# dernasherbrezon/sdr-server

Measured on AMD Instinct MI355X. Metric: input IQ Msamples/s processed (all clients), 2.016 Msps->48 kHz xlating FIR, higher is better.
Workload: dtype f32; 1 GPU; 1024 clients x 48 kHz off one 2.016 Msps cu8 stream, D=42, 505 taps, 262144-byte blocks (BASELINE configs[3]; N=1: the >=1000-client single-GPU target); clients_total=1024, clients_per_gpu=1024, blocks_per_call=8, mode=optimized, parallelism=single GPU, rccl_ranks=1, feed=xlating_multi (C host)

## Files before the change

### sdr-server_amd/csrc/xl_kernels.hip

```cpp
#include "xl_dev_inline.h"
#include "xl_chain_plan.h"

#include <hip/hip_ext.h>

#include <stdlib.h>

__global__ __launch_bounds__(64) void xl_nco_table_kernel(const XlNcoClient *__restrict__ cl, uint32_t n,
                                                          const float2 *state_in, float2 *state_out,
                                                          float2 *__restrict__ tab, const XlPos pos,
                                                          const uint32_t explicit_K, const uint32_t prio,
                                                          const uint32_t lanes) {
  if (prio == 3) __builtin_amdgcn_s_setprio(3);
  else if (prio == 2) __builtin_amdgcn_s_setprio(2);
  else if (prio == 1) __builtin_amdgcn_s_setprio(1);
  if (threadIdx.x >= lanes) return;
  const uint32_t c = blockIdx.x * lanes + threadIdx.x;
  if (c >= n) return;
  const XlNcoClient k = cl[c];
  const XlBnd bnd = xl_nco_bnd(k, pos, explicit_K);
  asm volatile("" ::: "v255", "a255");
  xl_nco_client_chain<true>(k, bnd, 0u, bnd.K, state_in, state_out, tab);
}

#define XLC_RING 64u
XL_DEV uint32_t xl_lds_off(const void *p) { return (uint32_t)(uintptr_t)(__attribute__((address_space(3))) const char *)p; }
XL_DEV void xl_lds_post(const uint32_t addr, const uint32_t v) { asm volatile("ds_write_b32 %0, %1" ::"v"(addr), "v"(v) : "memory"); }
XL_DEV void xl_lds_post64(const uint32_t addr, const v2f v) { asm volatile("ds_write_b64 %0, %1" ::"v"(addr), "v"(v) : "memory"); }
XL_DEV uint32_t xl_lds_poll(const uint32_t addr) {
  uint32_t v;
  asm volatile("ds_read_b32 %0, %1\n\ts_waitcnt lgkmcnt(0)" : "=v"(v) : "v"(addr) : "memory");
  return v;
}

XL_DEV uint32_t xl_lds_poll3_min(const uint32_t a0, const uint32_t a1, const uint32_t a2) {
  uint32_t v0, v1, v2;
  asm volatile("ds_read_b32 %0, %3\n\tds_read_b32 %1, %4\n\tds_read_b32 %2, %5\n\ts_waitcnt lgkmcnt(0)"
               : "=&v"(v0), "=&v"(v1), "=&v"(v2)
               : "v"(a0), "v"(a1), "v"(a2)
               : "memory");
  v0 = v0 < v1 ? v0 : v1;
  return v0 < v2 ? v0 : v2;
}
XL_DEV uint32_t xl_chain_lim(const uint32_t mn) { return mn >= 0x7FFFFFE0u ? 0xFFFFFFFFu : 2u * mn + XLC_RING; }
XL_DEV uint32_t xl_chain_wait_drained(const uint32_t upto, const uint32_t a0, const uint32_t a1, const uint32_t a2) {
  uint32_t lim = 0u;
  for (uint32_t spin = 0; spin < (1u << 22); ++spin) {
    lim = xl_chain_lim((uint32_t)__builtin_amdgcn_readfirstlane((int)xl_lds_poll3_min(a0, a1, a2)));
    if (upto <= lim) break;
    __builtin_amdgcn_s_sleep(1);
  }
  return lim;
}
XL_DEV uint32_t xl_chain_event(uint32_t ev) {
  const unsigned long long act = __ballot(ev != 0xFFFFFFFFu);
  if (act == 0ull) return 0xFFFFFFFFu;
  const uint32_t first = (uint32_t)__builtin_amdgcn_readlane((int)ev, (int)__ffsll((long long)act) - 1);
  if (__ballot(ev != 0xFFFFFFFFu && ev != first) == 0ull) return first;
#pragma unroll
  for (int sh = 1; sh < 64; sh <<= 1) {
    const uint32_t other = (uint32_t)__shfl_xor((int)ev, sh);
    ev = other < ev ? other : ev;
  }
  return (uint32_t)__builtin_amdgcn_readfirstlane((int)ev);
}

#define XLC_ALIGN ".p2align 6\n\t"
#define XLC_MUL "v_pk_mul_f32 %[t1], %[p], %[inc] op_sel_hi:[1,0]\n\tv_pk_mul_f32 %[t2], %[p], %[inc] op_sel:[0,1] op_sel_hi:[1,1]\n\t"
#define XLC_ADD "v_pk_add_f32 %[p], %[t1], %[t2] op_sel:[0,1] op_sel_hi:[1,0] neg_lo:[0,1]\n\t"
#define XLC_STEP XLC_MUL XLC_ADD
#define XLC_STEP2(I1, I2) XLC_MUL I1 "\n\t" XLC_ADD I2 "\n\t"
#define XLC_STEPS10 XLC_STEP XLC_STEP XLC_STEP XLC_STEP XLC_STEP XLC_STEP XLC_STEP XLC_STEP XLC_STEP XLC_STEP
#define XLC_ANY_LOOP                                                                       \
  "1:\n\t" XLC_MUL "ds_write_b64 %[addr], %[p]\n\t" XLC_ADD                               \
  XLC_STEP2("v_add_u32 %[cnt], 1, %[cnt]", "s_sub_u32 %[todo], %[todo], 1")               \
  XLC_MUL "ds_write_b32 %[paddr], %[cnt]\n\t" XLC_ADD                                     \
  XLC_MUL "v_add_u32 %[off], 0x200, %[off]\n\t" XLC_ADD                                   \
  XLC_MUL "v_and_b32 %[off], 0x7fff, %[off]\n\t" XLC_ADD                                  \
  XLC_STEP2("v_add_u32 %[addr], %[off], %[base]", "s_cmp_lg_u32 %[todo], 0")              \
  XLC_STEPS10 "s_cbranch_scc1 1b\n\t"
#define XLC_B8_LOOP                                                                        \
  "2:\n\t" XLC_E7("0", "512", "1024", "1536", "2048", "2560", "3072")                    \
  XLC_MUL "ds_write_b64 %[addr], %[p] offset:3584\n\t" XLC_ADD                           \
  XLC_STEP2("v_add_u32 %[cnt], 8, %[cnt]", "s_sub_u32 %[todo8], %[todo8], 1")            \
  XLC_MUL "ds_write_b32 %[paddr], %[cnt]\n\t" XLC_ADD                                    \
  XLC_MUL "v_add_u32 %[off], 0x1000, %[off]\n\t" XLC_ADD                                 \
  XLC_MUL "v_and_b32 %[off], 0x7fff, %[off]\n\t" XLC_ADD                                 \
  XLC_STEP2("v_add_u32 %[addr], %[off], %[base]", "s_cmp_lg_u32 %[todo8], 0")            \
  XLC_STEPS10 "s_cbranch_scc1 2b\n\t"
#define XLC_ANY_PART "s_cmp_eq_u32 %[todo], 0\n\ts_cbranch_scc1 3f\n\t" XLC_ANY_LOOP "3:\n\ts_nop 0\n\t"
#define XLC_B8_PART "s_cmp_eq_u32 %[todo8], 0\n\ts_cbranch_scc1 4f\n\t" XLC_B8_LOOP "4:\n\ts_nop 0\n\t"
#define XLC_STEP_LOOP "1:\n\t" XLC_STEP2("s_sub_u32 %[todo], %[todo], 1", "s_cmp_lg_u32 %[todo], 0") "s_cbranch_scc1 1b\n\t"
#define XLC_QENTRY(OFFS) XLC_MUL "ds_write_b64 %[addr], %[p] offset:" OFFS "\n\t" XLC_ADD XLC_STEP XLC_STEP
#define XLC_E(OFFS) XLC_QENTRY(OFFS) XLC_STEP XLC_STEP XLC_STEP XLC_STEPS10
#define XLC_E7(B0, B1, B2, B3, B4, B5, B6) XLC_E(B0) XLC_E(B1) XLC_E(B2) XLC_E(B3) XLC_E(B4) XLC_E(B5) XLC_E(B6)
#define XLC_E8(B0, B1, B2, B3, B4, B5, B6, B7) XLC_E7(B0, B1, B2, B3, B4, B5, B6) XLC_E(B7)
#define XLC_B32_LOOP                                                                                         \
  XLC_E8("0", "512", "1024", "1536", "2048", "2560", "3072", "3584")                                       \
  XLC_E8("4096", "4608", "5120", "5632", "6144", "6656", "7168", "7680")                                   \
  XLC_E8("8192", "8704", "9216", "9728", "10240", "10752", "11264", "11776")                               \
  XLC_E("12288") XLC_E("12800") XLC_E("13312") XLC_E("13824") XLC_E("14336") XLC_E("14848")               \
  XLC_QENTRY("15360")                                                                                      \
  XLC_MUL "ds_read_b32 %[mn], %[an0]\n\t" XLC_ADD                                                           \
  XLC_MUL "ds_read_b32 %[n1], %[an1]\n\t" XLC_ADD                                                           \
  XLC_MUL "ds_read_b32 %[n2], %[an2]\n\t" XLC_ADD XLC_STEPS10                                               \
  XLC_MUL "ds_write_b64 %[addr], %[p] offset:15872\n\t" XLC_ADD                                             \
  XLC_MUL "v_add_u32 %[cnt], 32, %[cnt]\n\t" XLC_ADD "s_sub_u32 %[todo], %[todo], 1\n\t"                    \
  XLC_MUL "ds_write_b32 %[paddr], %[cnt]\n\t" XLC_ADD                                                       \
  XLC_MUL "v_add_u32 %[off], 0x4000, %[off]\n\t" XLC_ADD                                                    \
  XLC_MUL "v_and_b32 %[off], 0x7fff, %[off]\n\t" XLC_ADD                                                    \
  XLC_STEP2("v_add_u32 %[addr], %[off], %[base]", "s_add_u32 %[need], %[need], 16")                         \
  XLC_STEP2("s_waitcnt lgkmcnt(0)", "v_min_u32 %[mn], %[mn], %[n1]")                                        \
  XLC_STEP2("v_min_u32 %[mn], %[mn], %[n2]", "s_nop 0")                                                     \
  XLC_STEP2("v_readfirstlane_b32 %[sm], %[mn]", "s_nop 0")                                                  \
  XLC_STEP2("s_cmp_ge_u32 %[sm], %[need]", "s_cselect_b32 %[st], %[todo], 0")                               \
  XLC_STEP XLC_STEP XLC_STEP XLC_STEP XLC_STEP XLC_STEP
static_assert(XL_PH_STRIDE == 16u && XLC_RING * 64u * 8u == 0x8000u, "the chain wave's asm blocks are written for 16 steps per entry and a 32 KB ring");

__global__ __launch_bounds__(256) void xl_nco_chain_kernel(const XlNcoClient *__restrict__ cl, uint32_t n,
                                                           const float2 *state_in, const XlChainCalls calls,
                                                           XlPos pos, unsigned long long *stats) {
  asm volatile("" ::: "v255", "a255");
  const unsigned long long t_entry = stats ? wall_clock64() : 0ull;
  __shared__ v2f ring[XLC_RING][64];
  __shared__ uint32_t s_emax;
  __shared__ uint32_t s_prod;
  __shared__ uint32_t s_next[3];
  const uint32_t w = __builtin_amdgcn_readfirstlane(threadIdx.x >> 6), lane = threadIdx.x & 63u;
  const uint32_t c = blockIdx.x * 64u + lane;
  const bool have = c < n;
  XlNcoClient k;
  k.incr = make_float2(1.0f, 0.0f);
  k.out_off = 0u, k.slot = 0u, k.D = 1u, k.rem0 = 0u;
  if (have) k = cl[c];
  v2f p = {1.0f, 0.0f};
  if (w == 0 && have) p = (v2f){state_in[k.slot].x, state_in[k.slot].y};
  unsigned long long cyc = 0ull, ticks = 0ull, wfirst = 0ull;
  uint32_t entries = 0u;
  for (uint32_t call = 0; call < calls.n; ++call, pos = xl_grid_next(pos)) {
    float2 *const tab = calls.tab[call];
    float2 *const state_out = calls.state_out[call];
    if (call) __syncthreads();
    XlBnd bnd = xl_nco_bnd(k, pos, 0xFFFFFFFFu);
    if (!have) bnd.K = 0u;
    const uint32_t K = bnd.K, E = (K + XL_PH_STRIDE - 1u) >> XL_PH_SHIFT;
    if (threadIdx.x == 0) {
      s_emax = 0u;
      s_prod = 0u;
      s_next[0] = 0u, s_next[1] = 1u, s_next[2] = 2u;
    }
    __syncthreads();
    if (w == 0 && E > 0u) atomicMax(&s_emax, E);
    __syncthreads();
    const uint32_t Emax = (uint32_t)__builtin_amdgcn_readfirstlane((int)s_emax);
    const uint32_t a_prod = xl_lds_off(&s_prod), a_ring0 = xl_lds_off(&ring[0][0]), a_ring = xl_lds_off(&ring[0][lane]);
    v2f *__restrict__ o = reinterpret_cast<v2f *>(tab) + (k.out_off >> XL_PH_SHIFT);
    if (w == 0) {
      __builtin_amdgcn_s_setprio(3);
      const v2f inc = {k.incr.x, k.incr.y};
      uint32_t nb = xl_bnd_next(bnd, 0u);
      const uint32_t a_n0 = xl_lds_off(&s_next[0]), a_n1 = xl_lds_off(&s_next[1]), a_n2 = xl_lds_off(&s_next[2]);
      const unsigned long long c0 = stats ? clock64() : 0ull, w0 = stats ? wall_clock64() : 0ull;
      unsigned long long t_region = 0ull, t_drain = 0ull, t_b32 = 0ull;
      uint32_t n_drain = 0u, n_b32 = 0u, n_event = 0u, n_runs = 0u;
      uint32_t e = 0;
      uint32_t lim = XLC_RING;
      uint32_t evs = xl_chain_event(0u < K ? (nb < K ? nb : K) : 0xFFFFFFFFu);
      while (e < Emax) {
        uint32_t e_stop = evs == 0u ? 0u : (evs - 1u) >> XL_PH_SHIFT;
        e_stop = e_stop < Emax ? e_stop : Emax;
        if (pos.pad & XL_POS_FMA_STEP) e_stop = e;
        const unsigned long long r0 = stats ? clock64() : 0ull;
        if ((e << XL_PH_SHIFT) < K) {
          const XlChainPlan8 pl = xl_chain_plan8(e, e_stop, XLC_RING, 32u, 8u);
          uint32_t ee = e;
          v2f t1, t2;
#define XLC_COVER_RUN(N1, N8, PARTS)                                                                                         \
  if ((N1) + (N8) != 0u) {                                                                                                   \
    uint32_t todo = (N1), todo8 = (N8);                                                                                      \
    const uint32_t total = todo + 8u * todo8;                                                                                \
    if (ee + total > lim) {                                                                                                  \
      const unsigned long long d0 = stats ? clock64() : 0ull;                                                                \
      lim = xl_chain_wait_drained(ee + total, a_n0, a_n1, a_n2);                                                             \
      if (stats) t_drain += clock64() - d0, ++n_drain;                                                                       \
    }                                                                                                                        \
    uint32_t off = ((ee & (XLC_RING - 1u)) << 9) + lane * (uint32_t)sizeof(v2f);     \
    uint32_t addr = a_ring0 + off, cnt = ee;                                                                                 \
    ee += total;                                                                                                             \
    asm volatile(XLC_ALIGN PARTS                                                                                             \
                 : [p] "+v"(p), [off] "+v"(off), [addr] "+v"(addr), [cnt] "+v"(cnt), [t1] "=&v"(t1), [t2] "=&v"(t2),         \
                   [todo] "+s"(todo), [todo8] "+s"(todo8)                                                                    \
                 : [inc] "v"(inc), [base] "v"(a_ring0), [paddr] "v"(a_prod)                                                  \
                 : "memory", "scc");                                                                                         \
  }
          XLC_COVER_RUN(pl.head1, pl.head8, XLC_ANY_PART XLC_B8_PART);
          for (uint32_t want = pl.blocks; want != 0u;) {
            if (ee + 32u > lim) {
              const unsigned long long d0 = stats ? clock64() : 0ull;
              lim = xl_chain_wait_drained(ee + 32u, a_n0, a_n1, a_n2);
              if (stats) t_drain += clock64() - d0, ++n_drain;
            }
            uint32_t off = ((ee & (XLC_RING - 1u)) << 9) + lane * (uint32_t)sizeof(v2f);
            uint32_t addr = a_ring0 + off, cnt = ee;
            uint32_t left = want, need = (ee >> 1) - 16u, mn, n1, n2, sm, st;
            const unsigned long long b0 = stats ? clock64() : 0ull;
            asm volatile(XLC_ALIGN "1:\n\t" XLC_B32_LOOP "s_cmp_lg_u32 %[st], 0\n\ts_cbranch_scc1 1b\n\t"
                         : [p] "+v"(p), [off] "+v"(off), [addr] "+v"(addr), [cnt] "+v"(cnt), [t1] "=&v"(t1), [t2] "=&v"(t2),
                           [mn] "=&v"(mn), [n1] "=&v"(n1), [n2] "=&v"(n2), [todo] "+s"(left), [need] "+s"(need), [sm] "=&s"(sm),
                           [st] "=&s"(st)
                         : [inc] "v"(inc), [base] "v"(a_ring0), [paddr] "v"(a_prod), [an0] "v"(a_n0), [an1] "v"(a_n1), [an2] "v"(a_n2)
                         : "memory", "scc");
            const uint32_t ran = (want - left) << 5;
            if (stats) t_b32 += clock64() - b0, n_b32 += ran, ++n_runs;
            lim = xl_chain_lim(sm);
            ee += ran;
            want = left;
          }
          XLC_COVER_RUN(pl.tail1, pl.tail8, XLC_B8_PART XLC_ANY_PART);
#undef XLC_COVER_RUN
        }
        if (e_stop > e) e = e_stop;
        if (stats) t_region += clock64() - r0, ++n_event;
        if (e < Emax) {
          if (e + 1u > lim) lim = xl_chain_wait_drained(e + 1u, a_n0, a_n1, a_n2);
          const uint32_t m0 = e << XL_PH_SHIFT;
          if (m0 < K) xl_lds_post64(a_ring + (e & (XLC_RING - 1u)) * 64u * (uint32_t)sizeof(v2f), p);
          xl_lds_post(a_prod, e + 1u);
          uint32_t m = m0;
          if (!(pos.pad & XL_POS_FMA_STEP) && evs - m0 - 1u < XL_PH_STRIDE &&
              __ballot(m0 < K && (nb != evs || m0 + XL_PH_STRIDE > K)) == 0ull && m0 < K) {
            v2f t1, t2;
            uint32_t todo = evs - m0;
            asm volatile(XLC_ALIGN XLC_STEP_LOOP
                         : [p] "+v"(p), [t1] "=&v"(t1), [t2] "=&v"(t2), [todo] "+s"(todo)
                         : [inc] "v"(inc)
                         : "scc");
            p = xl_nco_renorm(p);
            nb = xl_bnd_next(bnd, evs);
            m = evs;
            todo = m0 + XL_PH_STRIDE - evs;
            if (todo != 0u && __ballot(nb <= m0 + XL_PH_STRIDE) == 0ull) {
              asm volatile(XLC_ALIGN XLC_STEP_LOOP
                           : [p] "+v"(p), [t1] "=&v"(t1), [t2] "=&v"(t2), [todo] "+s"(todo)
                           : [inc] "v"(inc)
                           : "scc");
              m = m0 + XL_PH_STRIDE;
            }
          }
          for (; m < m0 + XL_PH_STRIDE && m < K; ++m) {
            p = xl_nco_next_any(p, inc, bnd.flags);
            if (m + 1u == nb) {
              p = xl_nco_renorm(p);
              nb = xl_bnd_next(bnd, m + 1u);
            }
          }
          ++e;
          evs = xl_chain_event((e << XL_PH_SHIFT) < K ? (nb < K ? nb : K) : 0xFFFFFFFFu);
        }
      }
      if (have) state_out[k.slot] = make_float2(p.x, p.y);
      if (stats) {
        cyc += clock64() - c0;
        const unsigned long long w1 = wall_clock64();
        ticks += w1 - w0;
        entries += Emax;
        if (call == 0u) wfirst = w0;
        if (lane == 0u && blockIdx.x < 1024u) {
          stats[8192u + 8u * blockIdx.x + 1u + 2u * call] = w0 - t_entry;
          stats[8192u + 8u * blockIdx.x + 2u + 2u * call] = w1 - t_entry;
        }
        if (lane == 0u && blockIdx.x < 128u) {
          unsigned long long *const sp = stats + 4096u + 32u * blockIdx.x + 8u * call;
          const unsigned long long k0 = clock64(), k1 = clock64(), k2 = clock64(), k3 = clock64(), k4 = clock64();
          (void)k1, (void)k2, (void)k3;
          sp[0] = k0 - c0, sp[1] = t_region, sp[2] = t_drain, sp[3] = t_b32;
          sp[4] = n_drain, sp[5] = n_b32, sp[6] = n_event | ((unsigned long long)n_runs << 32), sp[7] = (k4 - k0) / 4ull;
        }
      }
      continue;
    }
    const uint32_t j = w - 1u;
    const uint32_t a_next = xl_lds_off(&s_next[j]);
    v4f *__restrict__ o4 = reinterpret_cast<v4f *>(o);
    for (uint32_t q = j; 2u * q < Emax; q += 3u) {
      const uint32_t need = 2u * q + 2u < Emax ? 2u * q + 2u : Emax;
      for (uint32_t spin = 0; spin < (1u << 24); ++spin) {
        if (xl_lds_poll(a_prod) >= need) break;
        __builtin_amdgcn_s_sleep(1);
      }
      if (2u * q < E) {
        v2f a, b2 = {0.0f, 0.0f};
        const uint32_t ra = a_ring + ((2u * q) & (XLC_RING - 1u)) * 64u * (uint32_t)sizeof(v2f);
        const uint32_t rb = a_ring + ((2u * q + 1u) & (XLC_RING - 1u)) * 64u * (uint32_t)sizeof(v2f);
        const bool two = 2u * q + 1u < E;
        asm volatile("ds_read_b64 %0, %1" : "=v"(a) : "v"(ra) : "memory");
        if (two) asm volatile("ds_read_b64 %0, %1" : "=v"(b2) : "v"(rb) : "memory");
        asm volatile("s_waitcnt lgkmcnt(0)" ::: "memory");
        if (two) o4[q] = (v4f){a.x, a.y, b2.x, b2.y};
        else o[2u * q] = a;
      }
      xl_lds_post(a_next, q + 3u);
    }
    xl_lds_post(a_next, 0xFFFFFFFFu);
  }
  if (stats) __syncthreads();
  if (stats && threadIdx.x == 0u) {
    if (blockIdx.x < 1024u) {
      stats[8192u + 8u * blockIdx.x] = t_entry;
      stats[8192u + 8u * blockIdx.x + 7u] = wall_clock64() - t_entry;
    }
    stats[4u * blockIdx.x] = cyc;
    stats[4u * blockIdx.x + 1u] = ticks;
    stats[4u * blockIdx.x + 2u] = entries;
    stats[4u * blockIdx.x + 3u] = wfirst;
  }
}

template <int FMT>
XL_DEV void xl_stage_window(const XlFirArgs &a, const uint32_t zero_below, const uint32_t win0, const uint32_t wlen,
                            v2f *__restrict__ win) {
  const uint32_t bd = blockDim.x;
  for (uint32_t j0 = threadIdx.x; j0 < wlen; j0 += 4u * bd) {
    v2f v[4];
    bool ok[4];
#pragma unroll
    for (int u = 0; u < 4; ++u) {
      const uint32_t j = j0 + u * bd;
      const uint32_t s = win0 + j;
      const bool first = s < a.n0;
      ok[u] = j < wlen && s >= zero_below && (first || s - a.n0 < a.n1);
      const void *src = (first || !ok[u]) ? a.in0 : a.in1;
      const uint32_t idx = ok[u] ? (first ? s : s - a.n0) : 0u;
      v[u] = xl_sample(src, FMT, idx);
    }
#pragma unroll
    for (int u = 0; u < 4; ++u) {
      const uint32_t j = j0 + u * bd;
      if (j < wlen) win[j] = ok[u] ? v[u] : (v2f){0.0f, 0.0f};
    }
  }
}

template <int CT, int MODE, bool WIDE>
__global__ __launch_bounds__(64 * XL_NW_MAX) __attribute__((amdgpu_num_sgpr(96))) void xl_fir_kernel(const XlFirArgs a) {
  extern __shared__ __attribute__((aligned(16))) v2f xl_win[];
  const uint32_t OT = a.ota;

  if (blockIdx.x < a.nco_blocks) {
    if (((a.flags >> 4) & 3u) == 3u) __builtin_amdgcn_s_setprio(3);
    else if (((a.flags >> 4) & 3u) == 2u) __builtin_amdgcn_s_setprio(2);
    else if (((a.flags >> 4) & 3u) == 1u) __builtin_amdgcn_s_setprio(1);
    const uint32_t nwave = threadIdx.x >> 6, nlane = threadIdx.x & 63u;
    if (nwave < a.nco_wpw && nlane < XL_NCO_LANES) {
      const unsigned long long t0 = a.trace ? wall_clock64() : 0ull;
      const uint32_t c = (blockIdx.x * a.nco_wpw + nwave) * XL_NCO_LANES + nlane;
      if (c < a.nco_nclients) {
        const XlNcoClient k = a.nco_clients[c];
        const XlBnd bnd = xl_nco_bnd(k, xl_grid_next(a.pos), 0xFFFFFFFFu);
        xl_nco_client_chain<false>(k, bnd, 0u, bnd.K, a.nco_state_in, a.nco_state_out, a.nco_tab);
      }
      if (a.trace && nlane == 0) {
        unsigned long long *tn = a.trace + ((size_t)blockIdx.x * XL_NW_MAX + nwave) * 6;
        tn[0] = t0;
        tn[3] = wall_clock64();
        tn[4] = __builtin_amdgcn_s_getreg((4 << 0) | (0 << 6) | (31 << 11));
        tn[5] = __builtin_amdgcn_s_getreg((20 << 0) | (0 << 6) | (31 << 11));
      }
    }
    return;
  }

  if (!(a.flags & 2u)) __builtin_amdgcn_s_setprio(3);
  const uint32_t b = blockIdx.x - a.nco_blocks;
  const unsigned long long t_entry = a.trace ? wall_clock64() : 0ull;

  const uint32_t roll_blocks = gridDim.x - a.nco_blocks < XL_ROLL_BLOCKS ? gridDim.x - a.nco_blocks : XL_ROLL_BLOCKS;
  if (a.hist_out != nullptr && b < roll_blocks) {
    const uint16_t *__restrict__ h0 = reinterpret_cast<const uint16_t *>(a.in0);
    const uint16_t *__restrict__ h1 = reinterpret_cast<const uint16_t *>(a.in1);
    uint16_t *__restrict__ ho = reinterpret_cast<uint16_t *>(a.hist_out);
    const uint32_t hu = a.hist_units, nu = a.block_units;
    for (uint32_t j = b * blockDim.x + threadIdx.x; j < hu; j += roll_blocks * blockDim.x) {
      const uint32_t sidx = nu + j;
      ho[j] = (sidx < hu) ? h0[sidx] : h1[sidx - hu];
    }
  }
  const uint32_t xcd = b & 7u, idx = b >> 3;
  const uint32_t total = a.ngroups * a.xtiles;
  const uint32_t per = total >> 3, extra = total & 7u;
  const uint32_t len = per + (xcd < extra ? 1u : 0u);
  if (idx >= len) return;
  const uint32_t wi = xcd * per + (xcd < extra ? xcd : extra) + idx;
  const uint32_t y = wi / a.xtiles;
  const uint32_t x = wi - y * a.xtiles;
  if (y >= a.ngroups) return;

  const cu32_p g = (cu32_p)(uintptr_t)(a.groups + y);
  const uint32_t D = g[0], Tpad = g[2], ntiles = g[4];
  const XlDyn d = a.explicit_dyn ? a.dyn1 : xl_grid_dyn(D, g[1], g[3], g[7], a.pos);
  const uint32_t K = d.K;
  const bool live = x * OT < K;
  if (!live && a.nco_lanes == 0u) return;

  const uint32_t w = __builtin_amdgcn_readfirstlane(threadIdx.x >> 6);
  v2f phs[CT];
#pragma unroll
  for (int c = 0; c < CT; ++c) phs[c] = (v2f){1.0f, 0.0f};
  if (live) {
    if (w < ntiles) {
      constexpr uint32_t G = 64u / XL_PH_STRIDE;
      const uint32_t lane = threadIdx.x & 63u;
      v2f *__restrict__ pl = xl_win + w * (CT * 64u);
      const uint32_t *__restrict__ tg = reinterpret_cast<const uint32_t *>(a.groups + y) + 8u + w * XL_TILE_DWORDS;
      const uint32_t c = lane / G, e = lane % G;
      const uint32_t m0 = x * OT + e * XL_PH_STRIDE;
      if (c < tg[1] && e * XL_PH_STRIDE < OT && m0 < K) {
        const uint32_t off = tg[2 + c];
        const float2 ci = reinterpret_cast<const float2 *>(tg + 2 + XL_CT_MAX)[c];
        const uint32_t left = K - m0, span = OT < XL_PH_STRIDE ? OT : XL_PH_STRIDE;
        XlBnd bnd;
        bnd.j0 = d.j0, bnd.D = D, bnd.S = a.pos.S, bnd.G = a.explicit_dyn ? 1u : a.pos.G, bnd.K = K, bnd.flags = a.pos.pad;
        v2f *__restrict__ dst = pl + c * 64u + e * XL_PH_STRIDE;
        xl_phase_walk((reinterpret_cast<const v2f *>(a.phtab) + (off >> XL_PH_SHIFT))[m0 >> XL_PH_SHIFT], m0,
                      left < span ? left : span, (v2f){ci.x, ci.y}, bnd, [&](uint32_t i, v2f ph) { dst[i] = ph; });
      }
      __builtin_amdgcn_wave_barrier();
#pragma unroll
      for (int cc = 0; cc < CT; ++cc) phs[cc] = pl[cc * 64u + lane];
    }
    __syncthreads();

    const uint32_t win0 = d.base + x * OT * D;
    const uint32_t wlen = (OT - 1u) * D + Tpad;
    if (a.fmt == XLF_CU8) xl_stage_window<XLF_CU8>(a, d.zero_below, win0, wlen, xl_win);
    else if (a.fmt == XLF_CS8) xl_stage_window<XLF_CS8>(a, d.zero_below, win0, wlen, xl_win);
    else if (a.fmt == XLF_CS16) xl_stage_window<XLF_CS16>(a, d.zero_below, win0, wlen, xl_win);
    else xl_stage_window<XLF_CF32>(a, d.zero_below, win0, wlen, xl_win);
  }
  __syncthreads();

  if (w >= ntiles) {
    const uint32_t nlane = threadIdx.x & 63u;
    const uint32_t slot = (g[6] + (w - ntiles)) * a.xtiles + x;
    if (a.nco_lanes != 0u && slot < a.nco_slots && nlane < a.nco_lanes) {
      __builtin_amdgcn_s_setprio(3);
      const unsigned long long t0 = a.trace ? wall_clock64() : 0ull;
      const uint32_t c = slot * a.nco_lanes + nlane;
      if (c < a.nco_nclients) {
        const XlNcoClient k = a.nco_clients[c];
        const XlBnd bnd = xl_nco_bnd(k, xl_grid_next(a.pos), 0xFFFFFFFFu);
        xl_nco_client_chain<false>(k, bnd, 0u, bnd.K, a.nco_state_in, a.nco_state_out, a.nco_tab);
      }
      if (a.trace && nlane == 0) {
        unsigned long long *tn = a.trace + ((size_t)blockIdx.x * XL_NW_MAX + w) * 6;
        tn[0] = t0;
        tn[3] = wall_clock64();
        tn[4] = __builtin_amdgcn_s_getreg((4 << 0) | (0 << 6) | (31 << 11));
        tn[5] = __builtin_amdgcn_s_getreg((20 << 0) | (0 << 6) | (31 << 11));
      }
    }
    return;
  }
  if (!live) return;
  const uint32_t lane = threadIdx.x & 63u;
  unsigned long long *tr = a.trace ? a.trace + ((size_t)blockIdx.x * XL_NW_MAX + w) * 6 : nullptr;
  if (tr && lane == 0) {
    tr[0] = t_entry;
    tr[1] = wall_clock64();
    tr[4] = __builtin_amdgcn_s_getreg((4 << 0) | (0 << 6) | (31 << 11));
    tr[5] = __builtin_amdgcn_s_getreg((20 << 0) | (0 << 6) | (31 << 11));
  }
  const cu32_p t = g + 8 + w * XL_TILE_DWORDS;
  const uint32_t ncl = t[1];
  const cfloat_p tp = (cfloat_p)(uintptr_t)(a.taps + t[0]);

  XlAcc<MODE> acc[CT];
#pragma unroll
  for (int c = 0; c < CT; ++c) acc[c].clear();

  constexpr int STEP = (CT == 9 || CT == 10) ? 6 : 4;
  const v2f *lp = xl_win + (lane >= OT ? 0u : lane) * D;
#define XL_TAP_LOOP(I0, I1)                                                                       \
  for (uint32_t i = (I0); i < (I1); i += STEP) {                                                  \
    v2f xs[STEP];                                                                                 \
    if (WIDE) {                                                                                   \
      _Pragma("unroll") for (int u = 0; u < STEP; u += 2) {                                       \
        const v4f q = *reinterpret_cast<const v4f *>(lp + i + u);                                 \
        xs[u] = (v2f){q.x, q.y};                                                                  \
        xs[u + 1] = (v2f){q.z, q.w};                                                              \
      }                                                                                           \
    } else {                                                                                      \
      _Pragma("unroll") for (int u = 0; u < STEP; ++u) xs[u] = lp[i + u];                         \
    }                                                                                             \
    const cfloat_p tq = tp + (size_t)i * (2 * CT);                                                \
    _Pragma("unroll") for (int u = 0; u < STEP; ++u) {                                            \
      _Pragma("unroll") for (int c = 0; c < CT; ++c)                                              \
        acc[c].mac(xs[u], tq[(u * CT + c) * 2], tq[(u * CT + c) * 2 + 1]);                        \
    }                                                                                             \
  }
  if (a.flags & 2u) {
    XL_TAP_LOOP(0u, Tpad)
  } else {
    const uint32_t steps = Tpad / STEP;
    const uint32_t b1 = steps / 2, b2 = (7 * steps) / 8;
    const uint32_t e1 = b1 * STEP < Tpad ? b1 * STEP : Tpad;
    const uint32_t e2 = b2 * STEP < Tpad ? b2 * STEP : Tpad;
    __builtin_amdgcn_s_setprio(2);
    XL_TAP_LOOP(0u, e1)
    __builtin_amdgcn_s_setprio(1);
    XL_TAP_LOOP(e1, e2)
    __builtin_amdgcn_s_setprio(0);
    XL_TAP_LOOP(e2, Tpad)
    __builtin_amdgcn_s_setprio(3);
  }
#undef XL_TAP_LOOP

  if (tr && lane == 0) tr[2] = wall_clock64();
  v2f *__restrict__ out = reinterpret_cast<v2f *>(a.out);
  {
    const uint32_t m = x * OT + lane;
    if (m < K && lane < OT) {
#pragma unroll
      for (int c = 0; c < CT; ++c) {
        if ((uint32_t)c < ncl) out[t[2 + c] + m] = xl_rotate<MODE>(acc[c].value(), phs[c]);
      }
    }
  }
  if (tr && lane == 0) {
    __builtin_amdgcn_s_waitcnt(0);
    tr[3] = wall_clock64();
  }
}

size_t xl_fir_lds_bytes_ota(uint32_t D, uint32_t Tpad, uint32_t ota) {
  return ((size_t)(ota - 1u) * D + Tpad) * sizeof(v2f);
}

uint32_t xl_fir_pick_ota(uint32_t D, uint32_t Tpad, size_t budget) {
  for (uint32_t ota = 64; ota >= 8; ota >>= 1)
    if (xl_fir_lds_bytes_ota(D, Tpad, ota) <= budget) return ota;
  return 0;
}

template <int CT, int MODE, bool WIDE>
static hipError_t xl_fir_go2(int nw, const XlFirArgs &a, size_t lds, hipStream_t s) {
  static bool attr_done = false;
  if (!attr_done) {
    hipError_t e = hipFuncSetAttribute(reinterpret_cast<const void *>(&xl_fir_kernel<CT, MODE, WIDE>),
                                       hipFuncAttributeMaxDynamicSharedMemorySize, 160 * 1024);
    if (e != hipSuccess) return e;
    attr_done = true;
  }
  const uint32_t nblocks = a.nco_blocks + 8u * ((a.ngroups * a.xtiles + 7u) / 8u);
  if (nblocks == 0) return hipSuccess;
  const size_t need = (size_t)nw * CT * 64u * sizeof(float2);
  if (lds < need) lds = need;
  hipLaunchKernelGGL((xl_fir_kernel<CT, MODE, WIDE>), dim3(nblocks), dim3(64 * nw), lds, s, a);
  return hipGetLastError();
}

template <int CT, int MODE>
static hipError_t xl_fir_go(int nw, const XlFirArgs &a, size_t lds, hipStream_t s) {
  return (a.flags & 1u) ? xl_fir_go2<CT, MODE, true>(nw, a, lds, s) : xl_fir_go2<CT, MODE, false>(nw, a, lds, s);
}

hipError_t xl_launch_fir(int ct, int mode, int nw, const XlFirArgs &a, size_t lds, hipStream_t s) {
  if (lds > 160 * 1024 || nw < 1 || nw > XL_NW_MAX) return hipErrorInvalidValue;
  if (a.ota != 64 && a.ota != 32 && a.ota != 16 && a.ota != 8) return hipErrorInvalidValue;
  switch (ct * 2 + (mode ? 1 : 0)) {
    case 2: return xl_fir_go<1, 0>(nw, a, lds, s);
    case 3: return xl_fir_go<1, 1>(nw, a, lds, s);
    case 4: return xl_fir_go<2, 0>(nw, a, lds, s);
    case 5: return xl_fir_go<2, 1>(nw, a, lds, s);
    case 8: return xl_fir_go<4, 0>(nw, a, lds, s);
    case 9: return xl_fir_go<4, 1>(nw, a, lds, s);
    case 16: return xl_fir_go<8, 0>(nw, a, lds, s);
    case 17: return xl_fir_go<8, 1>(nw, a, lds, s);
    case 18: return xl_fir_go<9, 0>(nw, a, lds, s);
    case 19: return xl_fir_go<9, 1>(nw, a, lds, s);
    case 20: return xl_fir_go<10, 0>(nw, a, lds, s);
    case 21: return xl_fir_go<10, 1>(nw, a, lds, s);
    case 24: return xl_fir_go<12, 0>(nw, a, lds, s);
    case 25: return xl_fir_go<12, 1>(nw, a, lds, s);
    default: return hipErrorInvalidValue;
  }
}

hipError_t xl_launch_nco_table(const XlNcoClient *clients, uint32_t nclients, const float2 *state_in,
                               float2 *state_out, float2 *phtab, XlPos pos, uint32_t explicit_K, uint32_t prio,
                               hipStream_t s) {
  if (nclients == 0) return hipSuccess;
  const uint32_t lanes = XL_NCO_LANES;
  hipLaunchKernelGGL(xl_nco_table_kernel, dim3((nclients + lanes - 1) / lanes), dim3(64), 0, s, clients, nclients,
                     state_in, state_out, phtab, pos, explicit_K, prio, lanes);
  return hipGetLastError();
}

hipError_t xl_launch_nco_chain(const XlNcoClient *clients, uint32_t nclients, const float2 *state_in,
                               const XlChainCalls &calls, XlPos pos, unsigned long long *stats, hipStream_t s,
                               hipEvent_t done) {
  if (calls.n < 1u || calls.n > XL_CHAIN_MAXCALLS) return hipErrorInvalidValue;
  if (nclients == 0) return done ? hipEventRecord(done, s) : hipSuccess;
  if (done)
    hipExtLaunchKernelGGL(xl_nco_chain_kernel, dim3((nclients + 63u) / 64u), dim3(256), 0, s, nullptr, done, 0, clients,
                          nclients, state_in, calls, pos, stats);
  else
    hipLaunchKernelGGL(xl_nco_chain_kernel, dim3((nclients + 63u) / 64u), dim3(256), 0, s, clients, nclients, state_in,
                       calls, pos, stats);
  return hipGetLastError();
}

__global__ void xl_convert_cf32_kernel(const void *__restrict__ raw, int fmt, uint32_t n, v2f *__restrict__ dst) {
  for (uint32_t i = blockIdx.x * blockDim.x + threadIdx.x; i < n; i += gridDim.x * blockDim.x)
    dst[i] = xl_sample(raw, fmt, i);
}

hipError_t xl_launch_convert_cf32(const void *raw, int fmt, uint32_t nsamples, float2 *dst, hipStream_t s) {
  if (nsamples == 0) return hipSuccess;
  const uint32_t blocks = (nsamples + 255) / 256 < 2048 ? (nsamples + 255) / 256 : 2048;
  hipLaunchKernelGGL(xl_convert_cf32_kernel, dim3(blocks), dim3(256), 0, s, raw, fmt, nsamples,
                     reinterpret_cast<v2f *>(dst));
  return hipGetLastError();
}

__global__ void xl_convert_q15_kernel(const void *__restrict__ raw, int fmt, uint32_t n, int16_t *__restrict__ dst) {
  for (uint32_t i = blockIdx.x * blockDim.x + threadIdx.x; i < n; i += gridDim.x * blockDim.x) {
    int32_t v;
    if (fmt == XLF_CU8) {
      v = ((int32_t) reinterpret_cast<const uint8_t *>(raw)[i] - 128) * 256;
    } else if (fmt == XLF_CS8) {
      v = (int32_t) reinterpret_cast<const int8_t *>(raw)[i] * 256;
    } else {
      v = reinterpret_cast<const int16_t *>(raw)[i];
    }
    dst[i] = (int16_t)v;
  }
}

hipError_t xl_launch_convert_q15(const void *raw, int fmt, uint32_t nelems, int16_t *dst, hipStream_t s) {
  if (nelems == 0) return hipSuccess;
  const uint32_t blocks = (nelems + 255) / 256 < 2048 ? (nelems + 255) / 256 : 2048;
  hipLaunchKernelGGL(xl_convert_q15_kernel, dim3(blocks), dim3(256), 0, s, raw, fmt, nelems, dst);
  return hipGetLastError();
}

__global__ __launch_bounds__(1024) void xl_move_down_kernel(uint32_t *buf, uint32_t from_dw, uint32_t count_dw) {
  for (uint32_t base = 0; base < count_dw; base += 1024) {
    const uint32_t i = base + threadIdx.x;
    uint32_t v = 0;
    if (i < count_dw) v = buf[from_dw + i];
    __syncthreads();
    if (i < count_dw) buf[i] = v;
    __syncthreads();
  }
}

hipError_t xl_launch_move_down(void *buf, uint32_t from, uint32_t count, uint32_t elem_bytes, hipStream_t s) {
  if (count == 0 || from == 0) return hipSuccess;
  const uint32_t k = elem_bytes / 4;
  hipLaunchKernelGGL(xl_move_down_kernel, dim3(1), dim3(1024), 0, s, reinterpret_cast<uint32_t *>(buf), from * k,
                     count * k);
  return hipGetLastError();
}

__global__ void xl_update_history_kernel(const uint16_t *__restrict__ hist, const uint16_t *__restrict__ block,
                                         uint32_t h_u, uint32_t n_u, uint16_t *__restrict__ out) {
  for (uint32_t j = blockIdx.x * blockDim.x + threadIdx.x; j < h_u; j += gridDim.x * blockDim.x) {
    const uint32_t s = n_u + j;
    out[j] = (s < h_u) ? hist[s] : block[s - h_u];
  }
}

hipError_t xl_launch_update_history(const void *hist, const void *block, uint32_t h, uint32_t n, uint32_t bps,
                                    void *new_hist, hipStream_t s) {
  if (h == 0) return hipSuccess;
  const uint32_t u = bps / 2;
  const uint32_t hu = h * u, nu = n * u;
  const uint32_t blocks = (hu + 255) / 256 < 256 ? (hu + 255) / 256 : 256;
  hipLaunchKernelGGL(xl_update_history_kernel, dim3(blocks), dim3(256), 0, s, reinterpret_cast<const uint16_t *>(hist),
                     reinterpret_cast<const uint16_t *>(block), hu, nu, reinterpret_cast<uint16_t *>(new_hist));
  return hipGetLastError();
}


XL_DEV uint32_t xl_q15_step(const uint32_t p, const uint32_t a, const uint32_t b) {
  typedef short s2 __attribute__((ext_vector_type(2)));
  const int32_t tr = __builtin_amdgcn_sdot2(__builtin_bit_cast(s2, p), __builtin_bit_cast(s2, a), 0, false);
  const int32_t ti = __builtin_amdgcn_sdot2(__builtin_bit_cast(s2, p), __builtin_bit_cast(s2, b), 0, false);
  return __builtin_bit_cast(uint32_t, __builtin_amdgcn_cvt_pk_i16(tr >> 15, ti >> 15));
}

__global__ void xl_nco_table_q15_kernel(int32_t ir, int32_t ii, const short2 *state_in, short2 *state_out,
                                        uint32_t *__restrict__ tab, uint32_t K) {
  if (blockIdx.x != 0 || threadIdx.x != 0) return;
  const uint32_t a = ((uint32_t)ir & 0xFFFFu) | ((uint32_t)(-ii) << 16), b = ((uint32_t)ii & 0xFFFFu) | ((uint32_t)ir << 16);
  uint32_t p = ((uint32_t)(uint16_t)state_in->x) | ((uint32_t)(uint16_t)state_in->y << 16);
  uint32_t m = 0;
  for (; m + XL_PH_STRIDE <= K; m += XL_PH_STRIDE) {
    tab[m >> XL_PH_SHIFT] = p;
#pragma unroll
    for (uint32_t i = 0; i < XL_PH_STRIDE; ++i) p = xl_q15_step(p, a, b);
  }
  if (m < K) tab[m >> XL_PH_SHIFT] = p;
  for (; m < K; ++m) p = xl_q15_step(p, a, b);
  *state_out = make_short2((short)(p & 0xFFFFu), (short)(p >> 16));
}

hipError_t xl_launch_nco_table_q15(int16_t incr_re, int16_t incr_im, const short2 *state_in, short2 *state_out, short2 *phtab,
                                   uint32_t K, hipStream_t s) {
  if (K == 0) return hipSuccess;
  hipLaunchKernelGGL(xl_nco_table_q15_kernel, dim3(1), dim3(64), 0, s, (int32_t)incr_re, (int32_t)incr_im, state_in, state_out,
                     reinterpret_cast<uint32_t *>(phtab), K);
  return hipGetLastError();
}

__global__ __launch_bounds__(256) void xl_fir_q15_kernel(const uint32_t *__restrict__ work, const uint32_t *taps,
                                                         uint32_t T, uint32_t D, uint32_t K, int32_t ir, int32_t ii,
                                                         const uint32_t *__restrict__ phtab, short2 *__restrict__ out) {
  typedef short s2 __attribute__((ext_vector_type(2)));
  const uint32_t m = blockIdx.x * blockDim.x + threadIdx.x;
  if (m >= K) return;
  const uint32_t *__restrict__ w = work + (size_t)m * D;
  const cu32_p tq = (cu32_p)(uintptr_t)taps;
  long long sr = 0, si = 0;
  auto mac = [&](const uint32_t xv, const uint32_t hv) {
    const int32_t hr = (int16_t)(hv & 0xFFFFu), hi = (int32_t)hv >> 16;
    const int32_t xr = (int16_t)(xv & 0xFFFFu), xi = (int32_t)xv >> 16;
    const uint32_t swp = (hv >> 16) | (hv << 16);
    si += (long long)__builtin_amdgcn_sdot2(__builtin_bit_cast(s2, xv), __builtin_bit_cast(s2, swp), 0, false);
    sr += (long long)(xr * hr - xi * hi);
  };
  uint32_t i = 0;
  if ((((uintptr_t)w) & 7u) == 0u) {
    for (; i + 2u <= T; i += 2u) {
      const uint2 xv = *reinterpret_cast<const uint2 *>(w + i);
      mac(xv.x, tq[i]);
      mac(xv.y, tq[i + 1u]);
    }
  }
  for (; i < T; ++i) mac(w[i], tq[i]);
  const int32_t ar = xl_sat16((int32_t)(sr >> 15));
  const int32_t ai = xl_sat16((int32_t)(si >> 15));
  const uint32_t a = ((uint32_t)ir & 0xFFFFu) | ((uint32_t)(-ii) << 16), b = ((uint32_t)ii & 0xFFFFu) | ((uint32_t)ir << 16);
  uint32_t p = phtab[m >> XL_PH_SHIFT];
  for (uint32_t k = m & (XL_PH_STRIDE - 1u); k > 0u; --k) p = xl_q15_step(p, a, b);
  const int32_t pr = (int16_t)(p & 0xFFFFu), pi = (int32_t)p >> 16;
  const int32_t tr = ar * pr - ai * pi;
  const int32_t ti = ar * pi + ai * pr;
  out[m] = make_short2((short)xl_sat16(tr >> 15), (short)xl_sat16(ti >> 15));
}

hipError_t xl_launch_fir_q15(const short2 *work, const short2 *taps, uint32_t T, uint32_t D, uint32_t K, int16_t incr_re,
                             int16_t incr_im, const short2 *phtab, short2 *out, hipStream_t s) {
  if (K == 0) return hipSuccess;
  hipLaunchKernelGGL(xl_fir_q15_kernel, dim3((K + 63) / 64), dim3(64), 0, s, reinterpret_cast<const uint32_t *>(work),
                     reinterpret_cast<const uint32_t *>(taps), T, D, K, (int32_t)incr_re, (int32_t)incr_im,
                     reinterpret_cast<const uint32_t *>(phtab), out);
  return hipGetLastError();
}


__global__ __launch_bounds__(64) void xl_nco_q15_batch_kernel(const XlNcoClient *__restrict__ cl, const uint32_t *__restrict__ qinc,
                                                              uint32_t n, short2 *qstate, short2 *__restrict__ tab, const XlPos pos) {
  const uint32_t c = blockIdx.x * 64u + threadIdx.x;
  if (c >= n) return;
  const XlNcoClient k = cl[c];
  const uint32_t K = xl_nco_bnd(k, pos, 0xFFFFFFFFu).K;
  const int32_t ir = (int16_t)(qinc[c] & 0xFFFFu), ii = (int16_t)(qinc[c] >> 16);
  int32_t pr = qstate[k.slot].x, pi = qstate[k.slot].y;
  short2 *__restrict__ o = tab + (k.out_off >> XL_PH_SHIFT);
  for (uint32_t m = 0; m < K; ++m) {
    if ((m & (XL_PH_STRIDE - 1u)) == 0u) o[m >> XL_PH_SHIFT] = make_short2((short)pr, (short)pi);
    const int32_t tr = pr * ir - pi * ii, ti = pr * ii + pi * ir;
    pr = xl_sat16(tr >> 15);
    pi = xl_sat16(ti >> 15);
  }
  qstate[k.slot] = make_short2((short)pr, (short)pi);
}

hipError_t xl_launch_nco_q15_batch(const XlNcoClient *clients, const uint32_t *qinc, uint32_t nclients, short2 *qstate,
                                   short2 *qphtab, XlPos pos, hipStream_t s) {
  if (nclients == 0) return hipSuccess;
  hipLaunchKernelGGL(xl_nco_q15_batch_kernel, dim3((nclients + 63u) / 64u), dim3(64), 0, s, clients, qinc, nclients, qstate,
                     qphtab, pos);
  return hipGetLastError();
}

__global__ __launch_bounds__(64) void xl_nco_q15_ahead_kernel(const XlNcoClient *__restrict__ cl, const uint32_t *__restrict__ qinc,
                                                              uint32_t n, const short2 *__restrict__ state_src,
                                                              short2 *__restrict__ state_dst, uint32_t *__restrict__ tab,
                                                              const XlPos pos, const uint32_t prio) {
  if (prio == 3) __builtin_amdgcn_s_setprio(3);
  else if (prio == 2) __builtin_amdgcn_s_setprio(2);
  else if (prio == 1) __builtin_amdgcn_s_setprio(1);
  const uint32_t c = blockIdx.x * 64u + threadIdx.x;
  if (c >= n) return;
  const XlNcoClient k = cl[c];
  const uint32_t K = xl_nco_bnd(k, pos, 0xFFFFFFFFu).K;
  const uint32_t q = qinc[c];
  const int32_t ir = (int16_t)(q & 0xFFFFu), ii = (int16_t)(q >> 16);
  const uint32_t a = ((uint32_t)ir & 0xFFFFu) | ((uint32_t)(-ii) << 16), b = ((uint32_t)ii & 0xFFFFu) | ((uint32_t)ir << 16);
  const short2 p0 = state_src[k.slot];
  uint32_t p = ((uint32_t)(uint16_t)p0.x) | ((uint32_t)(uint16_t)p0.y << 16);
  uint32_t *__restrict__ o = tab + (k.out_off >> XL_PH_SHIFT);
  uint32_t m = 0;
  for (; m + XL_PH_STRIDE <= K; m += XL_PH_STRIDE) {
    o[m >> XL_PH_SHIFT] = p;
#pragma unroll
    for (uint32_t i = 0; i < XL_PH_STRIDE; ++i) p = xl_q15_step(p, a, b);
  }
  if (m < K) o[m >> XL_PH_SHIFT] = p;
  for (; m < K; ++m) p = xl_q15_step(p, a, b);
  state_dst[k.slot] = make_short2((short)(p & 0xFFFFu), (short)(p >> 16));
}

hipError_t xl_launch_nco_q15_ahead(const XlNcoClient *clients, const uint32_t *qinc, uint32_t nclients, const short2 *state_src,
                                   short2 *state_dst, short2 *qphtab, XlPos pos, uint32_t prio, hipStream_t s) {
  if (nclients == 0) return hipSuccess;
  hipLaunchKernelGGL(xl_nco_q15_ahead_kernel, dim3((nclients + 63u) / 64u), dim3(64), 0, s, clients, qinc, nclients, state_src,
                     state_dst, reinterpret_cast<uint32_t *>(qphtab), pos, prio);
  return hipGetLastError();
}

typedef const double __attribute__((address_space(4))) *cdouble_p;

template <int CT>
__global__ __launch_bounds__(64 * XL_NW_MAX) void xl_fir_q15_batch_kernel(const XlFirArgs a, const double *__restrict__ qtaps,
                                                                          const short2 *__restrict__ qphtab) {
  extern __shared__ __attribute__((aligned(16))) v2f xl_qwin[];
  const uint32_t OT = a.ota;
  const uint32_t b = blockIdx.x;
  const uint32_t roll_blocks = gridDim.x < XL_ROLL_BLOCKS ? gridDim.x : XL_ROLL_BLOCKS;
  if (a.hist_out != nullptr && b < roll_blocks) {
    const uint16_t *__restrict__ h0 = reinterpret_cast<const uint16_t *>(a.in0);
    const uint16_t *__restrict__ h1 = reinterpret_cast<const uint16_t *>(a.in1);
    uint16_t *__restrict__ ho = reinterpret_cast<uint16_t *>(a.hist_out);
    for (uint32_t j = b * blockDim.x + threadIdx.x; j < a.hist_units; j += roll_blocks * blockDim.x) {
      const uint32_t sidx = a.block_units + j;
      ho[j] = (sidx < a.hist_units) ? h0[sidx] : h1[sidx - a.hist_units];
    }
  }
  const uint32_t y = b / a.xtiles, x = b - y * a.xtiles;
  if (y >= a.ngroups) return;
  const cu32_p g = (cu32_p)(uintptr_t)(a.groups + y);
  const uint32_t D = g[0], T = g[1], Tpad = g[2], ntiles = g[4];
  const XlDyn d = xl_grid_dyn(D, T, g[3], g[7], a.pos);
  const uint32_t K = d.K;
  if (x * OT >= K) return;
  {
    const uint32_t win0 = d.base + x * OT * D, wlen = (OT - 1u) * D + Tpad;
    for (uint32_t j = threadIdx.x; j < wlen; j += blockDim.x) {
      const uint32_t sidx = win0 + j;
      const bool first = sidx < a.n0;
      const bool ok = sidx >= d.zero_below && (first || sidx - a.n0 < a.n1);
      const v2f v = xl_sample_q15((first || !ok) ? a.in0 : a.in1, a.fmt, ok ? (first ? sidx : sidx - a.n0) : 0u);
      xl_qwin[j] = ok ? v : (v2f){0.0f, 0.0f};
    }
  }
  __syncthreads();
  const uint32_t w = __builtin_amdgcn_readfirstlane(threadIdx.x >> 6), lane = threadIdx.x & 63u;
  if (w >= ntiles) return;
  const cu32_p t = g + 8 + w * XL_TILE_DWORDS;
  const uint32_t ncl = t[1];
  const cdouble_p tq = (cdouble_p)(uintptr_t)(qtaps + (size_t)t[0] * 2u);
  double accr[CT], acci[CT];
#pragma unroll
  for (int c = 0; c < CT; ++c) accr[c] = acci[c] = 0.0;
  const v2f *lp = xl_qwin + (lane >= OT ? 0u : lane) * D;
  for (uint32_t i = 0; i < T; ++i) {
    const v2f xs = lp[i];
    const double xr = (double)xs.x, xi = (double)xs.y;
    const cdouble_p h = tq + (size_t)i * (2 * CT);
#pragma unroll
    for (int c = 0; c < CT; ++c) {
      const double hr = h[2 * c], hi = h[2 * c + 1];
      accr[c] = __builtin_fma(xr, hr, accr[c]);
      accr[c] = __builtin_fma(-xi, hi, accr[c]);
      acci[c] = __builtin_fma(xr, hi, acci[c]);
      acci[c] = __builtin_fma(xi, hr, acci[c]);
    }
  }
  const uint32_t m = x * OT + lane;
  if (m >= K || lane >= OT) return;
#pragma unroll
  for (int c = 0; c < CT; ++c) {
    if ((uint32_t)c >= ncl) continue;
    const uint32_t off = t[2 + c], qi = t[2 + 3 * XL_CT_MAX + c];
    const int32_t ar = xl_q15_narrow_sum(accr[c]);
    const int32_t ai = xl_q15_narrow_sum(acci[c]);
    xl_q15_rotate_store(qphtab, a.out, off, qi, m, ar, ai);
  }
}

template <int CT>
static hipError_t xl_fir_q15_go(int nw, const XlFirArgs &a, const double *qtaps, const short2 *qphtab, size_t lds, hipStream_t s) {
  static bool attr_done = false;
  if (!attr_done) {
    hipError_t e = hipFuncSetAttribute(reinterpret_cast<const void *>(&xl_fir_q15_batch_kernel<CT>),
                                       hipFuncAttributeMaxDynamicSharedMemorySize, 160 * 1024);
    if (e != hipSuccess) return e;
    attr_done = true;
  }
  const uint32_t nblocks = a.ngroups * a.xtiles;
  if (nblocks == 0) return hipSuccess;
  hipLaunchKernelGGL((xl_fir_q15_batch_kernel<CT>), dim3(nblocks), dim3(64 * nw), lds, s, a, qtaps, qphtab);
  return hipGetLastError();
}

hipError_t xl_launch_fir_q15_batch(int ct, int nw, const XlFirArgs &a, const double *qtaps, const short2 *qphtab,
                                   size_t lds, hipStream_t s) {
  if (lds > 160 * 1024 || nw < 1 || nw > XL_NW_MAX) return hipErrorInvalidValue;
  switch (ct) {
    case 1: return xl_fir_q15_go<1>(nw, a, qtaps, qphtab, lds, s);
    case 2: return xl_fir_q15_go<2>(nw, a, qtaps, qphtab, lds, s);
    case 4: return xl_fir_q15_go<4>(nw, a, qtaps, qphtab, lds, s);
    case 8: return xl_fir_q15_go<8>(nw, a, qtaps, qphtab, lds, s);
    case 9: return xl_fir_q15_go<9>(nw, a, qtaps, qphtab, lds, s);
    case 10: return xl_fir_q15_go<10>(nw, a, qtaps, qphtab, lds, s);
    case 12: return xl_fir_q15_go<12>(nw, a, qtaps, qphtab, lds, s);
    default: return hipErrorInvalidValue;
  }
}
```

Measured before the change: 5.855 million Msamples/s.

## Remove per-call block barriers from NCO chain kernel using monotonic ring counters

Replaces the per-call __syncthreads and shared atomicMax for Emax with a wave-level max reduction, and makes the producer/consumer ring counters monotonic across calls via an ebase offset. The producer wave can start the next call as soon as the ring has drained, without waiting on block barriers. The final phase state is handed off through a double-buffered LDS slot that a consumer wave writes out. This is meant to remove barrier stalls between calls so consecutive calls overlap, at the cost of more complex counter arithmetic and a possible wraparound or deadlock risk.

```diff
diff --git a/sdr-server_amd/csrc/xl_kernels.hip b/sdr-server_amd/csrc/xl_kernels.hip
--- a/sdr-server_amd/csrc/xl_kernels.hip
+++ b/sdr-server_amd/csrc/xl_kernels.hip
@@ -41,11 +41,14 @@
   v0 = v0 < v1 ? v0 : v1;
   return v0 < v2 ? v0 : v2;
 }
-XL_DEV uint32_t xl_chain_lim(const uint32_t mn) { return mn >= 0x7FFFFFE0u ? 0xFFFFFFFFu : 2u * mn + XLC_RING; }
-XL_DEV uint32_t xl_chain_wait_drained(const uint32_t upto, const uint32_t a0, const uint32_t a1, const uint32_t a2) {
+XL_DEV uint32_t xl_chain_lim(const uint32_t mn, const uint32_t qbase) {
+  return mn < qbase ? 0u : (mn - qbase >= 0x7FFFFFE0u ? 0xFFFFFFFFu : 2u * (mn - qbase) + XLC_RING);
+}
+XL_DEV uint32_t xl_chain_call_entries(const uint32_t Emax) { return 2u * ((Emax >> 1) + 1u); }
+XL_DEV uint32_t xl_chain_wait_drained(const uint32_t upto, const uint32_t qbase, const uint32_t a0, const uint32_t a1, const uint32_t a2) {
   uint32_t lim = 0u;
   for (uint32_t spin = 0; spin < (1u << 22); ++spin) {
-    lim = xl_chain_lim((uint32_t)__builtin_amdgcn_readfirstlane((int)xl_lds_poll3_min(a0, a1, a2)));
+    lim = xl_chain_lim((uint32_t)__builtin_amdgcn_readfirstlane((int)xl_lds_poll3_min(a0, a1, a2)), qbase);
     if (upto <= lim) break;
     __builtin_amdgcn_s_sleep(1);
   }
@@ -62,6 +65,16 @@
     ev = other < ev ? other : ev;
   }
   return (uint32_t)__builtin_amdgcn_readfirstlane((int)ev);
+}
+XL_DEV uint32_t xl_chain_emax(uint32_t E) {
+  const uint32_t first = (uint32_t)__builtin_amdgcn_readfirstlane((int)E);
+  if (__ballot(E != first) == 0ull) return first;
+#pragma unroll
+  for (int sh = 1; sh < 64; sh <<= 1) {
+    const uint32_t other = (uint32_t)__shfl_xor((int)E, sh);
+    E = other > E ? other : E;
+  }
+  return (uint32_t)__builtin_amdgcn_readfirstlane((int)E);
 }
 
 #define XLC_ALIGN ".p2align 6\n\t"
@@ -122,7 +135,7 @@
   asm volatile("" ::: "v255", "a255");
   const unsigned long long t_entry = stats ? wall_clock64() : 0ull;
   __shared__ v2f ring[XLC_RING][64];
-  __shared__ uint32_t s_emax;
+  __shared__ v2f s_state[2][64];
   __shared__ uint32_t s_prod;
   __shared__ uint32_t s_next[3];
   const uint32_t w = __builtin_amdgcn_readfirstlane(threadIdx.x >> 6), lane = threadIdx.x & 63u;
@@ -136,34 +149,32 @@
   if (w == 0 && have) p = (v2f){state_in[k.slot].x, state_in[k.slot].y};
   unsigned long long cyc = 0ull, ticks = 0ull, wfirst = 0ull;
   uint32_t entries = 0u;
+  if (threadIdx.x == 0) {
+    s_prod = 0u;
+    s_next[0] = 0u, s_next[1] = 1u, s_next[2] = 2u;
+  }
+  __syncthreads();
+  const uint32_t a_prod = xl_lds_off(&s_prod), a_ring0 = xl_lds_off(&ring[0][0]), a_ring = xl_lds_off(&ring[0][lane]);
+  const uint32_t a_state = xl_lds_off(&s_state[0][lane]);
+  uint32_t ebase = 0u;
   for (uint32_t call = 0; call < calls.n; ++call, pos = xl_grid_next(pos)) {
     float2 *const tab = calls.tab[call];
     float2 *const state_out = calls.state_out[call];
-    if (call) __syncthreads();
-    XlBnd bnd = xl_nco_bnd(k, pos, 0xFFFFFFFFu);
-    if (!have) bnd.K = 0u;
-    const uint32_t K = bnd.K, E = (K + XL_PH_STRIDE - 1u) >> XL_PH_SHIFT;
-    if (threadIdx.x == 0) {
-      s_emax = 0u;
-      s_prod = 0u;
-      s_next[0] = 0u, s_next[1] = 1u, s_next[2] = 2u;
-    }
-    __syncthreads();
-    if (w == 0 && E > 0u) atomicMax(&s_emax, E);
-    __syncthreads();
-    const uint32_t Emax = (uint32_t)__builtin_amdgcn_readfirstlane((int)s_emax);
-    const uint32_t a_prod = xl_lds_off(&s_prod), a_ring0 = xl_lds_off(&ring[0][0]), a_ring = xl_lds_off(&ring[0][lane]);
-    v2f *__restrict__ o = reinterpret_cast<v2f *>(tab) + (k.out_off >> XL_PH_SHIFT);
+    const uint32_t qbase = ebase >> 1;
     if (w == 0) {
       __builtin_amdgcn_s_setprio(3);
+      XlBnd bnd = xl_nco_bnd(k, pos, 0xFFFFFFFFu);
+      if (!have) bnd.K = 0u;
+      const uint32_t Emax = xl_chain_emax((bnd.K + XL_PH_STRIDE - 1u) >> XL_PH_SHIFT);
+      const uint32_t K = bnd.K;
       const v2f inc = {k.incr.x, k.incr.y};
       uint32_t nb = xl_bnd_next(bnd, 0u);
       const uint32_t a_n0 = xl_lds_off(&s_next[0]), a_n1 = xl_lds_off(&s_next[1]), a_n2 = xl_lds_off(&s_next[2]);
+      uint32_t lim = call ? xl_chain_wait_drained(XLC_RING, qbase, a_n0, a_n1, a_n2) : XLC_RING;
       const unsigned long long c0 = stats ? clock64() : 0ull, w0 = stats ? wall_clock64() : 0ull;
       unsigned long long t_region = 0ull, t_drain = 0ull, t_b32 = 0ull;
       uint32_t n_drain = 0u, n_b32 = 0u, n_event = 0u, n_runs = 0u;
       uint32_t e = 0;
-      uint32_t lim = XLC_RING;
       uint32_t evs = xl_chain_event(0u < K ? (nb < K ? nb : K) : 0xFFFFFFFFu);
       while (e < Emax) {
         uint32_t e_stop = evs == 0u ? 0u : (evs - 1u) >> XL_PH_SHIFT;
@@ -180,11 +191,11 @@
     const uint32_t total = todo + 8u * todo8;                                                                                \
     if (ee + total > lim) {                                                                                                  \
       const unsigned long long d0 = stats ? clock64() : 0ull;                                                                \
-      lim = xl_chain_wait_drained(ee + total, a_n0, a_n1, a_n2);                                                             \
+      lim = xl_chain_wait_drained(ee + total, qbase, a_n0, a_n1, a_n2);                                                      \
       if (stats) t_drain += clock64() - d0, ++n_drain;                                                                       \
     }                                                                                                                        \
     uint32_t off = ((ee & (XLC_RING - 1u)) << 9) + lane * (uint32_t)sizeof(v2f);     \
-    uint32_t addr = a_ring0 + off, cnt = ee;                                                                                 \
+    uint32_t addr = a_ring0 + off, cnt = ebase + ee;                                                                         \
     ee += total;                                                                                                             \
     asm volatile(XLC_ALIGN PARTS                                                                                             \
                  : [p] "+v"(p), [off] "+v"(off), [addr] "+v"(addr), [cnt] "+v"(cnt), [t1] "=&v"(t1), [t2] "=&v"(t2),         \
@@ -196,12 +207,12 @@
           for (uint32_t want = pl.blocks; want != 0u;) {
             if (ee + 32u > lim) {
               const unsigned long long d0 = stats ? clock64() : 0ull;
-              lim = xl_chain_wait_drained(ee + 32u, a_n0, a_n1, a_n2);
+              lim = xl_chain_wait_drained(ee + 32u, qbase, a_n0, a_n1, a_n2);
               if (stats) t_drain += clock64() - d0, ++n_drain;
             }
             uint32_t off = ((ee & (XLC_RING - 1u)) << 9) + lane * (uint32_t)sizeof(v2f);
-            uint32_t addr = a_ring0 + off, cnt = ee;
-            uint32_t left = want, need = (ee >> 1) - 16u, mn, n1, n2, sm, st;
+            uint32_t addr = a_ring0 + off, cnt = ebase + ee;
+            uint32_t left = want, need = qbase + (ee >> 1) - 16u, mn, n1, n2, sm, st;
             const unsigned long long b0 = stats ? clock64() : 0ull;
             asm volatile(XLC_ALIGN "1:\n\t" XLC_B32_LOOP "s_cmp_lg_u32 %[st], 0\n\ts_cbranch_scc1 1b\n\t"
                          : [p] "+v"(p), [off] "+v"(off), [addr] "+v"(addr), [cnt] "+v"(cnt), [t1] "=&v"(t1), [t2] "=&v"(t2),
@@ -211,7 +222,7 @@
                          : "memory", "scc");
             const uint32_t ran = (want - left) << 5;
             if (stats) t_b32 += clock64() - b0, n_b32 += ran, ++n_runs;
-            lim = xl_chain_lim(sm);
+            lim = xl_chain_lim(sm, qbase);
             ee += ran;
             want = left;
           }
@@ -221,10 +232,10 @@
         if (e_stop > e) e = e_stop;
         if (stats) t_region += clock64() - r0, ++n_event;
         if (e < Emax) {
-          if (e + 1u > lim) lim = xl_chain_wait_drained(e + 1u, a_n0, a_n1, a_n2);
+          if (e + 1u > lim) lim = xl_chain_wait_drained(e + 1u, qbase, a_n0, a_n1, a_n2);
           const uint32_t m0 = e << XL_PH_SHIFT;
           if (m0 < K) xl_lds_post64(a_ring + (e & (XLC_RING - 1u)) * 64u * (uint32_t)sizeof(v2f), p);
-          xl_lds_post(a_prod, e + 1u);
+          xl_lds_post(a_prod, ebase + e + 1u);
           uint32_t m = m0;
           if (!(pos.pad & XL_POS_FMA_STEP) && evs - m0 - 1u < XL_PH_STRIDE &&
               __ballot(m0 < K && (nb != evs || m0 + XL_PH_STRIDE > K)) == 0ull && m0 < K) {
@@ -257,7 +268,9 @@
           evs = xl_chain_event((e << XL_PH_SHIFT) < K ? (nb < K ? nb : K) : 0xFFFFFFFFu);
         }
       }
-      if (have) state_out[k.slot] = make_float2(p.x, p.y);
+      xl_lds_post64(a_state + (call & 1u) * 64u * (uint32_t)sizeof(v2f), p);
+      xl_lds_post(a_prod, ebase + xl_chain_call_entries(Emax));
+      ebase += xl_chain_call_entries(Emax);
       if (stats) {
         cyc += clock64() - c0;
         const unsigned long long w1 = wall_clock64();
@@ -280,9 +293,15 @@
     }
     const uint32_t j = w - 1u;
     const uint32_t a_next = xl_lds_off(&s_next[j]);
+    XlBnd bnd = xl_nco_bnd(k, pos, 0xFFFFFFFFu);
+    if (!have) bnd.K = 0u;
+    const uint32_t E = (bnd.K + XL_PH_STRIDE - 1u) >> XL_PH_SHIFT;
+    const uint32_t Emax = xl_chain_emax(E);
+    const uint32_t ebase_next = ebase + xl_chain_call_entries(Emax), qnext = ebase_next >> 1;
+    v2f *__restrict__ o = reinterpret_cast<v2f *>(tab) + (k.out_off >> XL_PH_SHIFT);
     v4f *__restrict__ o4 = reinterpret_cast<v4f *>(o);
     for (uint32_t q = j; 2u * q < Emax; q += 3u) {
-      const uint32_t need = 2u * q + 2u < Emax ? 2u * q + 2u : Emax;
+      const uint32_t need = ebase + (2u * q + 2u < Emax ? 2u * q + 2u : Emax);
       for (uint32_t spin = 0; spin < (1u << 24); ++spin) {
         if (xl_lds_poll(a_prod) >= need) break;
         __builtin_amdgcn_s_sleep(1);
@@ -298,9 +317,19 @@
         if (two) o4[q] = (v4f){a.x, a.y, b2.x, b2.y};
         else o[2u * q] = a;
       }
-      xl_lds_post(a_next, q + 3u);
-    }
-    xl_lds_post(a_next, 0xFFFFFFFFu);
+      xl_lds_post(a_next, 2u * (q + 3u) < Emax ? qbase + q + 3u : qnext + j);
+    }
+    xl_lds_post(a_next, qnext + j);
+    if (j == 0u) {
+      for (uint32_t spin = 0; spin < (1u << 24); ++spin) {
+        if (xl_lds_poll(a_prod) >= ebase_next) break;
+        __builtin_amdgcn_s_sleep(1);
+      }
+      v2f ps;
+      asm volatile("ds_read_b64 %0, %1\n\ts_waitcnt lgkmcnt(0)" : "=v"(ps) : "v"(a_state + (call & 1u) * 64u * (uint32_t)sizeof(v2f)) : "memory");
+      if (have) state_out[k.slot] = make_float2(ps.x, ps.y);
+    }
+    ebase = ebase_next;
   }
   if (stats) __syncthreads();
   if (stats && threadIdx.x == 0u) {
```

After: 5.868 million Msamples/s, median of 2. No clear change (+0.2%).
